# mynameisfiber/baton

Measured on NVIDIA H100. Metric: federated local samples/sec (whole box), ResNet-18 FedAvg, synthetic non-IID 32x32 shards, higher is better.
Workload: dtype bf16

## Files before the change

baton_b200/csrc/bindings.cpp:

```cpp
#include <ATen/cuda/CUDAContext.h>
#include <c10/cuda/CUDAGuard.h>
#include <torch/extension.h>

#include <optional>
#include <vector>

#include "launch.h"

namespace {

inline cudaStream_t cur_stream() { return at::cuda::getCurrentCUDAStream().stream(); }
inline void check(int rc, const char* what) {
  TORCH_CHECK(rc == 0, "baton_b200::", what, " failed with code ", rc,
              rc > 0 ? std::string(" (") + cudaGetErrorString(static_cast<cudaError_t>(rc)) + ")" : std::string());
}
inline const void* cptr(const at::Tensor& t) { return t.data_ptr(); }
inline void* ptr(at::Tensor& t) { return t.data_ptr(); }
template <class T>
inline T* opt_ptr(const std::optional<at::Tensor>& t) {
  return (t.has_value() && t->defined()) ? reinterpret_cast<T*>(t->data_ptr()) : nullptr;
}
#define CHECK_CUDA(x) TORCH_CHECK((x).is_cuda(), #x " must be a CUDA tensor")

inline const float* prox_anchor(const std::optional<at::Tensor>& anchor, int64_t numel, const at::Tensor& hyper) {
// ... 239 lines not shown
                                static_cast<int>(stride), dgrad ? 1 : 0, static_cast<int>(mc), opt_ptr<float>(col_stats),
                                cur_stream());
  if (rc == -2) return false;
  check(rc, "conv_halo");
  return true;
}
bool conv_igemm_dgrad_s2(const at::Tensor& dy, const at::Tensor& w, at::Tensor dx, int64_t kh, int64_t kw,
                         const std::vector<int64_t>& ntaps, const std::vector<int64_t>& taps, int64_t force_bn) {
  CHECK_CUDA(dy); CHECK_CUDA(w); CHECK_CUDA(dx);
  TORCH_CHECK(dy.scalar_type() == at::kBFloat16 && w.scalar_type() == at::kBFloat16 && dx.scalar_type() == at::kBFloat16 &&
              dy.dim() == 4 && dx.dim() == 4 && dy.is_contiguous() && w.is_contiguous() && dx.is_contiguous());
  TORCH_CHECK(ntaps.size() == 4 && taps.size() == 16, "conv_igemm_dgrad_s2: 4 classes x 4 taps");
  int nt[4], tw[16];
  for (int i = 0; i < 4; ++i) nt[i] = static_cast<int>(ntaps[i]);
  for (int i = 0; i < 16; ++i) tw[i] = static_cast<int>(taps[i]);
  const c10::cuda::CUDAGuard guard(dy.device());
  const int rc = b200_conv_igemm_dgrad_s2(cptr(dy), cptr(w), ptr(dx), static_cast<int>(dx.size(0)),
                                          static_cast<int>(dx.size(1)), static_cast<int>(dx.size(2)),
                                          static_cast<int>(dx.size(3)), static_cast<int>(dy.size(3)), static_cast<int>(kh),
                                          static_cast<int>(kw), static_cast<int>(dy.size(1)), static_cast<int>(dy.size(2)),
                                          nt, tw, static_cast<int>(force_bn), cur_stream());
  if (rc == -2) return false;
  check(rc, "conv_igemm_dgrad_s2");
  return true;
}
bool conv_igemm_wgrad(const at::Tensor& dy, const at::Tensor& x, at::Tensor dw, int64_t cout, int64_t kh, int64_t kw,
                      int64_t stride, int64_t pad, int64_t ho, int64_t wo, int64_t split_k, int64_t force_bn,
                      const std::optional<at::Tensor>& sgd_theta, const std::optional<at::Tensor>& sgd_theta_bf16,
                      const std::optional<at::Tensor>& sgd_mom, const std::optional<at::Tensor>& sgd_hyper,
                      bool sgd_nesterov, const std::optional<at::Tensor>& sgd_anchor,
                      const std::optional<at::Tensor>& sgd_corr, const std::optional<at::Tensor>& sgd_v) {
  CHECK_CUDA(dy); CHECK_CUDA(x); CHECK_CUDA(dw);
  TORCH_CHECK(x.scalar_type() == at::kBFloat16 && dy.scalar_type() == at::kBFloat16 && dw.scalar_type() == at::kFloat &&
              x.dim() == 4 && x.is_contiguous() && dy.is_contiguous());
  const c10::cuda::CUDAGuard guard(x.device());
  const std::optional<B200SgdEpilogue> sgd =
      sgd_epilogue(sgd_theta, sgd_theta_bf16, sgd_mom, sgd_hyper, sgd_nesterov, sgd_anchor, sgd_corr, sgd_v);
  const int rc = b200_conv_igemm_wgrad(cptr(dy), cptr(x), dw.data_ptr<float>(), static_cast<int>(x.size(0)),
                                       static_cast<int>(x.size(1)), static_cast<int>(x.size(2)), static_cast<int>(x.size(3)),
                                       static_cast<int>(cout), static_cast<int>(kh), static_cast<int>(kw),
                                       static_cast<int>(stride), static_cast<int>(pad), static_cast<int>(ho),
                                       static_cast<int>(wo), static_cast<int>(split_k), static_cast<int>(force_bn),
                                       sgd ? &*sgd : nullptr, cur_stream());
  if (rc == -2 || rc == B200_SGD_EPILOGUE_DECLINED) return false;
  check(rc, "conv_igemm_wgrad");
  return true;
// ... 886 lines not shown
  const c10::cuda::CUDAGuard guard(pred.device());
  const int in32 = pred.scalar_type() == at::kFloat;
  const int out32 = dpred.has_value() && dpred->defined() && dpred->scalar_type() == at::kFloat;
  check(b200_mse(pred.data_ptr(), in32, target.data_ptr<float>(), opt_ptr<void>(dpred), out32,
                 loss_acc.data_ptr<float>(), pred.numel(), static_cast<float>(grad_scale), cur_stream()),
        "mse");
}

}

PYBIND11_MODULE(TORCH_EXTENSION_NAME, m) {
  m.doc() = "baton_b200 sm_90a kernels";
  m.attr("MAX_RANKS") = B200_MAX_RANKS;
  m.def("gemm", &gemm);
  m.def("trace_set", &trace_set);
  m.def("attention_fwd", &attention_fwd);
  m.def("attention_bwd", &attention_bwd);
  m.def("bn_bwd_cluster", &bn_bwd_cluster);
  m.def("im2col_tma_probe", &im2col_tma_probe);
  m.def("conv_igemm_fwd", &conv_igemm_fwd);
  m.def("conv_igemm_wgrad", &conv_igemm_wgrad);
  m.def("conv_igemm_dgrad", &conv_igemm_dgrad);
  m.def("conv_igemm_dgrad_s2", &conv_igemm_dgrad_s2);
  m.def("conv_halo", &conv_halo);
  m.def("gemm_batched", &gemm_batched);
  m.def("gemm_fp8", &gemm_fp8);
  m.def("quant_mx_rows", &quant_mx_rows);
  m.def("quant_mx_cols", &quant_mx_cols);
  m.def("fused_sgd", &fused_sgd);
  m.def("fused_sgd_segments", &fused_sgd_segments);
  m.def("weighted_sum", &weighted_sum);
  m.def("fold_client", &fold_client);
  m.def("scaffold_corr", &scaffold_corr);
  m.def("scaffold_dc", &scaffold_dc);
  m.def("cast", &cast);
  m.def("gather_rows", &gather_rows);
  m.def("gather_augment", &gather_augment);
  m.def("gather_mix", &gather_mix);
  m.def("colsum", &colsum);
  m.def("add_bf16", &add_bf16);
  m.def("relu_bwd", &relu_bwd);
  m.def("gelu", &gelu);
  m.def("gelu_bwd", &gelu_bwd);
  m.def("pad_rows", &pad_rows);
  m.def("embedding_bwd", &embedding_bwd);
  m.def("fedavg_allreduce", &fedavg_allreduce);
// ... 41 lines not shown
```

baton_b200/csrc/gemm_wgmma.cu:

```cuda
#define B200_TU_TAG 1
#include "ptx.cuh"
#include "epilogue.cuh"
#include "launch.h"
#include "pdl.cuh"
#include "sgd.cuh"

namespace b200 {

constexpr int BM = 128;
constexpr int BK = 64;
constexpr int WG_K = 16;
constexpr int GEMM_THREADS = 384;
constexpr int CONSUMER_WARPS = 8;
constexpr int CONSUMER_THREADS = 32 * CONSUMER_WARPS;
constexpr int MAX_STAGES = 8;
constexpr int S2_MAX_TAPS = 4;

struct GemmParams {
  int M, N, K;
  void* D;
  long long ldd;
  const float* bias;
  int out_fp32;
  int act;
// ... 339 lines not shown
  return w;
}
__device__ __forceinline__ int s2_dx_row(const GemmParams& p, int cls, int m) {
  if (m >= p.M) return -1;
  const int hw = p.conv_ho * p.conv_wo;
  const int n = m / hw, r = m - n * hw;
  const int i = r / p.conv_wo, j = r - i * p.conv_wo;
  const int h = 2 * i + (cls >> 1), w = 2 * j + (cls & 1);
  return (h < p.conv_h && w < p.conv_w) ? (n * p.conv_h + h) * p.conv_w + w : -1;
}
template <int BN>
__device__ __forceinline__ void s2_load_ktile(const CUtensorMap* tmA, const CUtensorMap* tmB, const GemmParams& p,
                                              uint8_t* sa, uint8_t* sb, uint64_t* bar, int cls, int kt, int m0, int n0) {
  const int cblocks = p.conv_cin >> 6;
  const int slot = kt / cblocks, cb = kt - slot * cblocks;
  const int tw = s2_tap(p, cls, slot);
  const int q0 = m0 % p.conv_wo, t0 = m0 / p.conv_wo;
  tma_load_im2col_4d(sa, tmA, bar, cb * 64, q0, t0 % p.conv_ho, t0 / p.conv_ho, (tw >> 24) & 0xff, (tw >> 16) & 0xff);
  const int wcol = (tw & 0xffff) * p.conv_ncol + n0;
#pragma unroll
  for (int j = 0; j < BN / 64; ++j) tma_load_2d(sb + j * 8192, tmB, bar, wcol + j * 64, cb * 64);
}

template <int BN, int STAGES, int CONV = 0, bool SGD = false, bool AFFINE = false, bool PROX = false, bool SCAF = false,
          bool ADAM = false>
__global__ void __launch_bounds__(GEMM_THREADS, 1)
gemm_bf16_fixed_kernel(const __grid_constant__ CUtensorMap tmA, const __grid_constant__ CUtensorMap tmB,
                         const GemmParams p) {
  using L = SmemLayout<BN>;
  static_assert(STAGES * L::STAGE_BYTES >= L::PART_BYTES, "the drained ring must hold the fp32 accumulator tile");
  extern __shared__ __align__(1024) uint8_t smem_raw[];
  uint8_t* smem = reinterpret_cast<uint8_t*>((reinterpret_cast<uintptr_t>(smem_raw) + 1023) & ~uintptr_t(1023));
  uint64_t* full_bar = reinterpret_cast<uint64_t*>(smem + STAGES * L::STAGE_BYTES);
  uint64_t* empty_bar = full_bar + STAGES;
  float* cstat = reinterpret_cast<float*>(empty_bar + STAGES);

  griddep_launch_dependents();
  const int warp = threadIdx.x >> 5;
  int m0 = blockIdx.y * BM;
  const int cls = CONV == 4 ? s2_class(p, m0) : 0;
  const int n0 = blockIdx.x * BN;
  const int k_tiles_total = CONV == 4 ? s2_ntaps(p, cls) * (p.conv_cin >> 6) : (p.K + BK - 1) / BK;
  const int bz_outer = p.batched ? static_cast<int>(blockIdx.z) / p.batch_inner : 0;
  const int bz_inner = p.batched ? static_cast<int>(blockIdx.z) % p.batch_inner : 0;
  const int kt_begin = p.batched ? 0 : blockIdx.z * p.k_tiles_per_split;
  int kt_end = kt_begin + p.k_tiles_per_split;
  if (kt_end > k_tiles_total) kt_end = k_tiles_total;
  const int num_kt = kt_end - kt_begin;

  if (warp == 0 && elect_one()) {
    tma_prefetch_desc(&tmA);
    tma_prefetch_desc(&tmB);
    for (int s = 0; s < STAGES; ++s) {
      mbar_init(&full_bar[s], 1);
      mbar_init(&empty_bar[s], CONSUMER_WARPS);
    }
    fence_barrier_init();
  }
  __syncthreads();
  griddep_wait();

  if (warp == 0) {
    if (elect_one()) {
      if (p.tile_flags != nullptr) {
        const int rows_here = (p.N - n0) < BN ? (p.N - n0) : BN;
// ... 17 lines not shown
        if constexpr (CONV == 2) {
          const int live = (p.N - n0 + 63) / 64 < BN / 64 ? (p.N - n0 + 63) / 64 : BN / 64;
          mbar_expect_tx(&full_bar[s], L::A_BYTES + live * 8192);
        } else {
          mbar_expect_tx(&full_bar[s], L::STAGE_BYTES);
        }
        if (p.batched) {
          if (!p.a_mn) {
            tma_load_4d(sa, &tmA, &full_bar[s], k0, m0, bz_inner, bz_outer);
          } else {
#pragma unroll
            for (int j = 0; j < BM / 64; ++j)
              tma_load_4d(sa + j * 8192, &tmA, &full_bar[s], m0 + j * 64, k0, bz_inner, bz_outer);
          }
          if (!p.b_mn) {
            tma_load_4d(sb, &tmB, &full_bar[s], k0, n0, bz_inner, bz_outer);
          } else {
#pragma unroll
            for (int j = 0; j < BN / 64; ++j)
              tma_load_4d(sb + j * 8192, &tmB, &full_bar[s], n0 + j * 64, k0, bz_inner, bz_outer);
          }
        } else if constexpr (CONV == 4) {
          s2_load_ktile<BN>(&tmA, &tmB, p, sa, sb, &full_bar[s], cls, kt_begin + i, m0, n0);
        } else {
        if constexpr (CONV == 1 || CONV == 3) {
          const int kt = kt_begin + i;
          const int cblocks = p.conv_cin >> 6;
          const int tap = kt / cblocks, cb = kt - tap * cblocks;
          const int fr = tap / p.conv_kw, fs = tap - fr * p.conv_kw;
          const int q0 = m0 % p.conv_wo, t0 = m0 / p.conv_wo;
          tma_load_im2col_4d(sa, &tmA, &full_bar[s], cb * 64, q0 * p.conv_stride - p.conv_pad,
                             (t0 % p.conv_ho) * p.conv_stride - p.conv_pad, t0 / p.conv_ho, fs, fr);
        } else if (!p.a_mn) {
          tma_load_2d(sa, &tmA, &full_bar[s], k0, m0);
        } else {
#pragma unroll
          for (int j = 0; j < BM / 64; ++j)
            tma_load_2d(sa + j * 8192, &tmA, &full_bar[s], m0 + j * 64, k0);
        }
        if constexpr (CONV == 2) {
          const int q0 = k0 % p.conv_wo, t0 = k0 / p.conv_wo;
          const int w0 = q0 * p.conv_stride - p.conv_pad, h0 = (t0 % p.conv_ho) * p.conv_stride - p.conv_pad;
          const int img = t0 / p.conv_ho;
#pragma unroll
          for (int j = 0; j < BN / 64; ++j) {
            const int col = n0 + j * 64;
// ... 15 lines not shown
        } else {
#pragma unroll
          for (int j = 0; j < BN / 64; ++j) tma_load_2d(sb + j * 8192, &tmB, &full_bar[s], n0 + j * 64, k0);
        }
        }
      }
    }
  } else if (warp >= 4) {
    const int ew = warp - 4;
    float acc[BN / 2];
    int s = 0;
    uint32_t ph = 0;
    consume_ktiles<BN>(acc, smem, STAGES, full_bar, empty_bar, s, ph, num_kt, p.a_mn, p.b_mn, ew >> 2);
    if (threadIdx.x == 128) TRACE_POINT();
    named_bar_sync(1, CONSUMER_THREADS);
    float* part = reinterpret_cast<float*>(smem);
    wg_store_acc<BN>(acc, part, L::PART_PITCH, 64 * (ew >> 2));
    named_bar_sync(1, CONSUMER_THREADS);
    const int q = ew & 3;
    constexpr int NCHUNK = BN / 32;
    const int c_begin = (ew < 4 ? 0 : (NCHUNK + 1) / 2) * 32, c_end = (ew < 4 ? (NCHUNK + 1) / 2 : NCHUNK) * 32;
    const int lrow = q * 32 + static_cast<int>(lane_id());
    const int row = m0 + lrow;
    const int orow = CONV == 4 ? s2_dx_row(p, cls, row) : row;
    const bool row_ok = CONV == 4 ? orow >= 0 : row < p.M;
    const size_t elt = p.out_fp32 ? 4 : 2;
    uint8_t* drow = reinterpret_cast<uint8_t*>(p.D) +
                    (static_cast<size_t>(CONV == 4 && orow < 0 ? 0 : orow) * p.ldd + static_cast<size_t>(bz_outer) * p.d_outer +
                     static_cast<size_t>(bz_inner) * p.d_inner) * elt;
    const bool vec_ok = ((reinterpret_cast<uintptr_t>(p.D) & 15) == 0) && ((p.ldd * elt) % 16 == 0);
    const bool sgd_vec = SGD && (p.ldd % 4 == 0) &&
                         ((reinterpret_cast<uintptr_t>(p.sgd_theta) | reinterpret_cast<uintptr_t>(p.sgd_mom) |
                           (PROX ? reinterpret_cast<uintptr_t>(p.sgd_anchor) : 0) |
                           (SCAF ? reinterpret_cast<uintptr_t>(p.sgd_corr) : 0) |
                           (ADAM ? reinterpret_cast<uintptr_t>(p.sgd_v) : 0)) & 15) == 0 &&
                         (reinterpret_cast<uintptr_t>(p.sgd_wb) & 7) == 0;
    float* sstat = cstat + q * 2 * BN;
    const bool want_stats = p.col_stats != nullptr;
#pragma unroll 1
    for (int c = c_begin; c < c_end; c += 32) {
      uint32_t r[32];
      acc_ld_row32(part + lrow * L::PART_PITCH + c, r);
      const int col0 = n0 + c;
      float v[32];
#pragma unroll
      for (int j = 0; j < 32; ++j) v[j] = __uint_as_float(r[j]);
      if (col0 >= p.N) {
        if (want_stats) { sstat[c + lane_id()] = 0.f; sstat[BN + c + lane_id()] = 0.f; }
        continue;
      }
      if constexpr (AFFINE) {
// ... 230 lines not shown
      epilogue_tile<BN>(p, acc_tile, ew & 3, ew >> 2, m0, n0, epi_stage + ew * EPI_WARP_BYTES,
                        vec_ok && ((d_off * elt) & 15) == 0, d_off);
    }
  }
}


template <int BN, bool CLUSTER, int CONV = 0, bool AFFINE = false>
__global__ void __launch_bounds__(GEMM_THREADS, 1)
gemm_bf16_splitk_kernel(const __grid_constant__ CUtensorMap tmA, const __grid_constant__ CUtensorMap tmB,
                        const GemmParams p) {
  using L = SmemLayout<BN>;
  extern __shared__ __align__(1024) uint8_t smem_raw[];
  uint8_t* smem = reinterpret_cast<uint8_t*>((reinterpret_cast<uintptr_t>(smem_raw) + 1023) & ~uintptr_t(1023));
  const int STAGES = p.stages;
  const int ring_bytes = STAGES * L::STAGE_BYTES;
  const int data_bytes = L::PART_BYTES > ring_bytes ? L::PART_BYTES : ring_bytes;
  uint64_t* full_bar = reinterpret_cast<uint64_t*>(smem + data_bytes);
  uint64_t* empty_bar = full_bar + MAX_STAGES;
  float* cstat = reinterpret_cast<float*>(empty_bar + MAX_STAGES);

  griddep_launch_dependents();
  const int warp = threadIdx.x >> 5;
  const int m0 = blockIdx.y * BM;
  const int n0 = blockIdx.x * BN;
  const int k_tiles_total = (p.K + BK - 1) / BK;
  const int kt_begin = blockIdx.z * p.k_tiles_per_split;
  int kt_end = kt_begin + p.k_tiles_per_split;
  if (kt_end > k_tiles_total) kt_end = k_tiles_total;
  const int num_kt = kt_end - kt_begin;

  if (warp == 0 && elect_one()) {
    tma_prefetch_desc(&tmA);
    tma_prefetch_desc(&tmB);
    for (int s = 0; s < STAGES; ++s) {
      mbar_init(&full_bar[s], 1);
      mbar_init(&empty_bar[s], CONSUMER_WARPS);
    }
    fence_barrier_init();
  }
  __syncthreads();
  griddep_wait();

  if (warp == 0) {
    if (elect_one()) {
      if (p.tile_flags != nullptr) {
        const int rows_here = (p.N - n0) < BN ? (p.N - n0) : BN;
        const uint32_t need = p.flag_epoch_ptr != nullptr ? *reinterpret_cast<const volatile uint32_t*>(p.flag_epoch_ptr)
                                                          : p.flag_epoch;
        wait_arrival_flags(p.tile_flags, p.flag_elem_off + static_cast<long long>(n0) * p.ldb,
                           p.flag_elem_off + static_cast<long long>(n0 + rows_here) * p.ldb - 1, p.flag_tile_elems, need);
        if (p.flag_bias_off >= 0)
          wait_arrival_flags(p.tile_flags, p.flag_bias_off + n0, p.flag_bias_off + n0 + rows_here - 1,
                             p.flag_tile_elems, need);
        fence_proxy_async_all();
      }
      int s = 0;
      uint32_t ph = 0;
      for (int i = 0; i < num_kt; ++i) {
        mbar_wait(&empty_bar[s], ph ^ 1);
        uint8_t* sa = smem + s * L::STAGE_BYTES;
        uint8_t* sb = sa + L::A_BYTES;
        const int k0 = (kt_begin + i) * BK;
        mbar_expect_tx(&full_bar[s], L::STAGE_BYTES);
        if constexpr (CONV == 1 || CONV == 3) {
          const int kt = kt_begin + i;
          const int cblocks = p.conv_cin >> 6;
          const int tap = kt / cblocks, cb = kt - tap * cblocks;
          const int fr = tap / p.conv_kw, fs = tap - fr * p.conv_kw;
          const int q0 = m0 % p.conv_wo, t0 = m0 / p.conv_wo;
          tma_load_im2col_4d(sa, &tmA, &full_bar[s], cb * 64, q0 * p.conv_stride - p.conv_pad,
                             (t0 % p.conv_ho) * p.conv_stride - p.conv_pad, t0 / p.conv_ho, fs, fr);
        } else if (!p.a_mn) {
          tma_load_2d(sa, &tmA, &full_bar[s], k0, m0);
        } else {
#pragma unroll
          for (int j = 0; j < BM / 64; ++j)
            tma_load_2d(sa + j * 8192, &tmA, &full_bar[s], m0 + j * 64, k0);
        }
        if constexpr (CONV == 3) {
          const int kt = kt_begin + i;
          const int cblocks = p.conv_cin >> 6;
          const int tap = kt / cblocks, cb = kt - tap * cblocks;
          const int wcol = (p.conv_taps - 1 - tap) * p.conv_ncol + n0;
#pragma unroll
          for (int j = 0; j < BN / 64; ++j) tma_load_2d(sb + j * 8192, &tmB, &full_bar[s], wcol + j * 64, cb * 64);
        } else if (!p.b_mn) {
// ... 12 lines not shown
    uint32_t ph = 0;
    consume_ktiles<BN>(acc, smem, STAGES, full_bar, empty_bar, s, ph, num_kt, p.a_mn, p.b_mn, ew >> 2);
    named_bar_sync(1, CONSUMER_THREADS);
    float* part = reinterpret_cast<float*>(smem);
    wg_store_acc<BN>(acc, part, L::PART_PITCH, 64 * (ew >> 2));
    if constexpr (!CLUSTER) {
      named_bar_sync(1, CONSUMER_THREADS);
      const int q = ew & 3;
      constexpr int NCHUNK = BN / 32;
      const int c_begin = (ew < 4 ? 0 : (NCHUNK + 1) / 2) * 32, c_end = (ew < 4 ? (NCHUNK + 1) / 2 : NCHUNK) * 32;
      const int lrow = q * 32 + static_cast<int>(lane_id());
      const int row = m0 + lrow;
      const size_t elt = p.out_fp32 ? 4 : 2;
      const bool vec_ok = ((reinterpret_cast<uintptr_t>(p.D) & 15) == 0) && ((p.ldd * elt) % 16 == 0);
#pragma unroll 1
      for (int c = c_begin; c < c_end; c += 32) {
        const int col0 = n0 + c;
        if (row >= p.M || col0 >= p.N) continue;
        uint32_t r[32];
        acc_ld_row32(part + lrow * L::PART_PITCH + c, r);
        float v[32];
#pragma unroll
        for (int j = 0; j < 32; ++j) v[j] = __uint_as_float(r[j]);
        store_row_chunk<32, AFFINE>(p, row, col0, v, vec_ok);
      }
    }
  }

  if constexpr (CLUSTER) {
    const int S = p.cluster_k;
    cluster_sync_all();
    if (warp >= 4 && warp < 8) {
      const uint32_t me = cluster_ctarank();
      const int rows_per = BM / S;
      constexpr int CG = BN / 8;
      const int t = threadIdx.x - 128;
      const size_t elt = p.out_fp32 ? 4 : 2;
      const bool vec_ok = ((reinterpret_cast<uintptr_t>(p.D) & 15) == 0) && ((p.ldd * elt) % 16 == 0);
      const bool want_stats = p.col_stats != nullptr;
      float cs[8] = {0.f, 0.f, 0.f, 0.f, 0.f, 0.f, 0.f, 0.f}, cq[8] = {0.f, 0.f, 0.f, 0.f, 0.f, 0.f, 0.f, 0.f};
      for (int item = t; item < rows_per * CG; item += 128) {
        const int lrow = static_cast<int>(me) * rows_per + item / CG;
        const int c = (item % CG) * 8;
        const uint32_t laddr = smem_u32(smem) + static_cast<uint32_t>((lrow * L::PART_PITCH + c) * 4);
        float v[8] = {0.f, 0.f, 0.f, 0.f, 0.f, 0.f, 0.f, 0.f};
        for (int r = 0; r < S; ++r) {
          const float4 a = ld_dsmem_f4(laddr, r), b = ld_dsmem_f4(laddr + 16, r);
          v[0] += a.x; v[1] += a.y; v[2] += a.z; v[3] += a.w;
          v[4] += b.x; v[5] += b.y; v[6] += b.z; v[7] += b.w;
        }
        const int row = m0 + lrow, col0 = n0 + c;
        if (want_stats) {
#pragma unroll
          for (int j = 0; j < 8; ++j) {
            const float rnd = __bfloat162float(__float2bfloat16_rn(v[j]));
            cs[j] += rnd;
            cq[j] = fmaf(rnd, rnd, cq[j]);
          }
        }
        if (row < p.M && col0 < p.N) store_row_chunk<8, AFFINE>(p, row, col0, v, vec_ok);
      }
      if (want_stats) {
#pragma unroll
        for (int j = 0; j < 8; ++j) {
#pragma unroll
          for (int o = CG; o < 32; o <<= 1) {
            cs[j] += __shfl_xor_sync(0xffffffffu, cs[j], o);
            cq[j] += __shfl_xor_sync(0xffffffffu, cq[j], o);
          }
        }
        const int wq = t >> 5, ln = t & 31;
        if (ln < CG) {
#pragma unroll
          for (int j = 0; j < 8; ++j) {
            cstat[wq * 2 * BN + ln * 8 + j] = cs[j];
            cstat[wq * 2 * BN + BN + ln * 8 + j] = cq[j];
          }
        }
        named_bar_sync(2, 128);
        for (int i = t; i < 2 * BN; i += 128) {
          const int col = i < BN ? i : i - BN;
          if (n0 + col < p.N) {
            const float v = cstat[i] + cstat[2 * BN + i] + cstat[4 * BN + i] + cstat[6 * BN + i];
// ... 467 lines not shown
  }
  if (max_taps == 0) return -2;
  const int bn = clamp_bn(force_bn > 0 ? force_bn : (Cin > 64 ? 128 : 64));
  CUtensorMap ta, tb;
  int rc = b200_encode_map_im2col_bf16(&ta, dy, N, Ho, Wo, Cout, 1, 1, 1, 0, 64, BM);
  if (rc) return rc;
  rc = make_map(&tb, w, Cout, static_cast<long long>(KH) * KW * Cin, static_cast<long long>(KH) * KW * Cin, 64, BK);
  if (rc) return rc;
  const int k_tiles = max_taps * (Cout / 64);
  p.M = static_cast<int>(M); p.N = Cin; p.K = k_tiles * BK; p.D = dx; p.ldd = Cin; p.bias = nullptr; p.out_fp32 = 0;
  p.act = 0; p.a_mn = 0; p.b_mn = 1; p.k_tiles_per_split = k_tiles; p.cluster_k = 1; p.atomic_out = 0;
  p.col_stats = nullptr;
  p.tile_flags = nullptr; p.flag_epoch = 0; p.alpha = 1.0f; p.flag_elem_off = 0; p.flag_tile_elems = 0;
  p.ldb = static_cast<long long>(KH) * KW * Cin;
  p.flag_bias_off = -1; p.flag_epoch_ptr = nullptr;
  p.batched = 0; p.batch_inner = 1; p.batch_count = 1; p.d_outer = 0; p.d_inner = 0;
  p.conv_ho = Ho; p.conv_wo = Wo; p.conv_stride = 2; p.conv_pad = 0; p.conv_kw = KW; p.conv_cin = Cout;
  p.conv_taps = KH * KW; p.conv_ncol = Cin; p.conv_h = H; p.conv_w = W;
  dim3 grid((Cin + bn - 1) / bn, static_cast<unsigned>(4 * tiles_m), 1);
  if (bn == 128) return launch_fixed<128, 6, 4>(ta, tb, p, grid, stream);
  return launch_fixed<64, 8, 4>(ta, tb, p, grid, stream);
}

extern "C" int b200_conv_igemm_wgrad(const void* dy, const void* x, float* dw, int N, int H, int W, int Cin, int Cout,
                                     int KH, int KW, int stride, int pad, int Ho, int Wo, int split_k, int force_bn,
                                     const B200SgdEpilogue* sgd, cudaStream_t stream) {
  using namespace b200;
  const long long Mp = static_cast<long long>(N) * Ho * Wo;
  const int Kc = KH * KW * Cin;
  if (Mp <= 0 || Cout <= 0) return 0;
  if (Cin % 64 != 0 || Cout % 8 != 0 || Mp > (1ll << 30) || (reinterpret_cast<uintptr_t>(x) & 15) ||
      (reinterpret_cast<uintptr_t>(dy) & 15) || (reinterpret_cast<uintptr_t>(dw) & 15))
    return -2;
  const int bn = clamp_bn(force_bn > 0 ? force_bn : (Kc > 64 ? 128 : 64));
  CUtensorMap ta, tb;
  int rc = make_map(&ta, dy, Mp, Cout, Cout, 64, BK);
  if (rc) return rc;
  rc = b200_encode_map_im2col_bf16(&tb, x, N, H, W, Cin, KH, KW, stride, pad, 64, 64);
  if (rc) return rc;
  const int k_tiles = static_cast<int>((Mp + BK - 1) / BK);
  if (split_k < 1) split_k = 1;
  if (split_k > k_tiles) split_k = k_tiles;
  const int per = (k_tiles + split_k - 1) / split_k;
  split_k = (k_tiles + per - 1) / per;
  if (sgd != nullptr && split_k != 1) return B200_SGD_EPILOGUE_DECLINED;
  GemmParams p;
// ... 21 lines not shown
```

baton_b200/csrc/launch.h:

```cpp
#pragma once
#include <cuda_runtime.h>
#include <stdint.h>

#define B200_MAX_RANKS 16

extern "C" {

struct B200SgdEpilogue {
  float* theta;
  void* theta_bf16;
  float* mom;
  const float* hyper;
  int nesterov;
  const float* anchor;
  const float* corr;
  float* v;
};
#define B200_SGD_EPILOGUE_DECLINED (-6)

struct B200AffineEpilogue {
  const float* scale;
  const float* shift;
  const void* residual;
  long long ldr;
// ... 1 lines not shown
};
#define B200_AFFINE_EPILOGUE_DECLINED (-7)

int b200_gemm_bf16(const void* a, const void* b, void* d, const float* bias, int M, int N, int K, long long lda,
                   long long ldb, long long ldd, int a_mn, int b_mn, int out_fp32, int act, int split_k, int accumulate,
                   float alpha, const uint32_t* tile_flags, uint32_t flag_epoch, long long flag_elem_off, int flag_tile_elems,
                   long long flag_bias_off, int force_bn, float* col_stats, const uint32_t* flag_epoch_ptr,
                   const B200SgdEpilogue* sgd, const B200AffineEpilogue* affine, cudaStream_t stream);
int b200_gemm_bf16_batched(const void* a, const void* b, void* d, int M, int N, int K, long long lda, long long ldb,
                           long long ldd, int a_mn, int b_mn, int out_fp32, int act, float alpha, int n_outer,
                           int n_inner, long long a_outer, long long a_inner, long long b_outer, long long b_inner,
                           long long d_outer, long long d_inner, int accumulate, cudaStream_t stream);
int b200_attention_fwd(const void* qkv, void* out, void* probs, int B, int S, int H, int dh, float scale,
                       cudaStream_t stream);
int b200_attention_bwd(const void* qkv, const void* dout, const void* probs, void* dqkv, int B, int S, int H, int dh,
                       float scale, cudaStream_t stream);
int b200_conv_igemm_fwd(const void* x, const void* w, void* y, int N, int H, int W, int Cin, int Cout, int KH, int KW,
                        int stride, int pad, int Ho, int Wo, int cluster_k, int force_bn, float* col_stats,
                        const B200AffineEpilogue* affine, cudaStream_t stream);
int b200_conv_igemm_dgrad(const void* dy, const void* w, void* dx, int N, int H, int W, int Cin, int Cout, int KH, int KW,
                          int pad, int Ho, int Wo, int cluster_k, int force_bn, cudaStream_t stream);
int b200_conv_igemm_dgrad_s2(const void* dy, const void* w, void* dx, int N, int H, int W, int Cin, int Cout, int KH,
                             int KW, int Ho, int Wo, const int* ntaps, const int* taps, int force_bn, cudaStream_t stream);
int b200_conv_igemm_wgrad(const void* dy, const void* x, float* dw, int N, int H, int W, int Cin, int Cout, int KH, int KW,
                          int stride, int pad, int Ho, int Wo, int split_k, int force_bn, const B200SgdEpilogue* sgd,
                          cudaStream_t stream);
int b200_conv_halo(const void* src, const void* w, void* out, int N, int H, int W, int C, int Nout, int stride,
                   int dgrad, int mc, float* col_stats, cudaStream_t stream);
int b200_im2col_tma_probe(const void* x, void* col, int N, int H, int W, int C, int KH, int KW, int stride, int pad,
                          int Ho, int Wo, cudaStream_t stream);
int b200_gemm_fp8(const void* a, const void* b, void* d, const float* bias, const void* sfa, const void* sfb, int M, int N,
                  int K, long long lda, long long ldb, long long ldd, int out_fp32, int act, int split_k, int accumulate,
                  float alpha, cudaStream_t stream);
int b200_quant_mx_rows(const void* x, void* q, void* sf, long long R, int C, long long ld_in, int Cp, cudaStream_t stream);
int b200_quant_mx_cols(const void* x, void* q, void* sf, long long R, int C, long long ld_in, long long Rp,
                       cudaStream_t stream);
int b200_gemm_simt(const void* a, const void* b, void* d, const float* bias, int M, int N, int K, long long lda,
                   long long ldb, long long ldd, int a_mn, int b_mn, int out_fp32, int act, int accumulate,
                   float alpha, cudaStream_t stream);

int b200_fused_sgd(float* w, float* g, float* mom, void* w_bf16, long long n, const float* hyper, int zero_grad,
                   int nesterov, const unsigned long long* wire_slot, const float* pack_global,
                   const float* pack_scale, long long n_pack, int wire_fp32, const float* prox_anchor,
                   const float* corr, float* adam_v, cudaStream_t stream);
int b200_fused_sgd_segments(float* w, float* g, float* mom, void* w_bf16, const long long* segments, int n_seg,
                            const float* hyper, int nesterov, const float* prox_anchor, const float* corr,
// ... 192 lines not shown
```

baton_b200/ops/functional.py:

```python
from __future__ import annotations

import collections
import functools
from typing import List, Optional, Sequence, Tuple

import torch

from ._ext import load

BF16 = torch.bfloat16
NUM_SMS = 132


def _pitch(t: torch.Tensor) -> int:
    assert t.dim() == 2 and (t.stride(1) == 1 or t.shape[1] == 1), "GEMM operand must have unit inner stride"
    return t.stride(0) if t.shape[0] > 1 else max(t.stride(0), t.shape[1])


def _tma_ok(t: torch.Tensor) -> bool:
    return t.dtype == BF16 and _pitch(t) % 8 == 0 and t.data_ptr() % 16 == 0


def pick_bn(M: int, N: int) -> int:
    m_tiles = (M + 127) // 128
# ... 387 lines not shown


def halo_smem_bytes(h: int, w: int, c: int = 64, stride: int = 1) -> int:
    ho, wo = conv_out_size(h, 3, stride, 1), conv_out_size(w, 3, stride, 1)
    box = (HALO_BM // (ho * wo)) * (stride * (ho - 1) + 3) * (stride * (wo - 1) + 3) * 128
    k_tiles = 9 * (c // 64)
    return c // 64 * round_up(box, 1024) + k_tiles * 8192 + round_up(1 + k_tiles, 16) * 8 + 4 * 64 * 4 + 1024


def halo_eligible(kh: int, kw: int, stride: int, pad: int, c: int, h: int, w: int,
                  affine: Optional[dict] = None, dgrad: bool = False) -> bool:
    if kh != 3 or kw != 3 or pad != 1 or (stride, c) not in _HALO_FORMS or (dgrad and stride != 1):
        return False
    hw = conv_out_size(h, 3, stride, 1) * conv_out_size(w, 3, stride, 1)
    return (hw <= HALO_BM and HALO_BM % hw == 0 and affine is None and
            halo_smem_bytes(h, w, c, stride) <= _HALO_MAX_SMEM)


def halo_cluster(m_rows: int) -> int:
    tiles = (m_rows + HALO_BM - 1) // HALO_BM
    return 4 if tiles % 4 == 0 else 2 if tiles % 2 == 0 else 1


def _conv_path(path: Optional[str], eligible: bool) -> str:
    if path is None:
        return "halo" if eligible else "im2col"
    if path not in ("halo", "im2col"):
        raise ValueError("path must be None, 'halo' or 'im2col', not {!r}".format(path))
    if path == "halo" and not eligible:
        raise ValueError("the halo kernel does not take this convolution (see halo_eligible)")
    return path


def conv_igemm_fwd(x: torch.Tensor, w2d: torch.Tensor, kh: int, kw: int, stride: int, pad: int,
                   col_stats: Optional[torch.Tensor] = None, affine: Optional[dict] = None,
                   cluster_k: Optional[int] = None, force_bn: int = 0,
                   out: Optional[torch.Tensor] = None, path: Optional[str] = None,
                   mc: Optional[int] = None) -> Optional[torch.Tensor]:
    n, h, w, c = x.shape
    cout = w2d.shape[0]
    if c % 64 or w2d.shape[1] != kh * kw * c or not x.is_contiguous() or not w2d.is_contiguous():
        return None
    ho, wo = conv_out_size(h, kh, stride, pad), conv_out_size(w, kw, stride, pad)
    M, K = n * ho * wo, kh * kw * c
    halo = halo_eligible(kh, kw, stride, pad, c, h, w, affine) and cout % 8 == 0
    if _conv_path(path, halo) == "halo":
        y = out if out is not None else torch.empty((M, cout), dtype=BF16, device=x.device)
        if not load().conv_halo(x, w2d, y, stride, False, mc or halo_cluster(M), col_stats):
            raise RuntimeError("conv_halo declined a convolution halo_eligible admits")
        return y
    bn = force_bn or pick_bn(M, cout)
    if cluster_k is None:
        cluster_k = pick_cluster_k(M, cout, K, bn)
    y = out if out is not None else torch.empty((M, cout), dtype=BF16, device=x.device)
    af = affine or {}
    ok = load().conv_igemm_fwd(x, w2d, y, kh, kw, stride, pad, ho, wo, cluster_k, bn, col_stats, af.get("scale"),
                               af.get("shift"), af.get("residual"), bool(af.get("relu", False)))
    return y if ok else None


S2_MAX_TAPS = 4


def conv_s2_dgrad_taps(kh: int, kw: int, pad: int, ho: int, wo: int) -> Optional[List[List[Tuple[int, int, int]]]]:
    classes = []
    for a in (0, 1):
        for b in (0, 1):
            taps = []
            for r in range(kh):
                if (a + pad - r) % 2:
                    continue
                dp = (a + pad - r) // 2
                for s in range(kw):
                    if (b + pad - s) % 2:
                        continue
                    dq = (b + pad - s) // 2
                    if dp < 0 or dq < 0:
                        return None
                    if dp < ho and dq < wo:
                        taps.append((r * kw + s, dp, dq))
            if len(taps) > S2_MAX_TAPS:
                return None
            classes.append(taps)
    return classes


def conv_igemm_dgrad(dy: torch.Tensor, w2d: torch.Tensor, in_shape, kh: int, kw: int, pad: int, stride: int = 1,
                     out: Optional[torch.Tensor] = None, path: Optional[str] = None,
                     mc: Optional[int] = None, cluster_k: Optional[int] = None) -> Optional[torch.Tensor]:
    n, h, w, c = in_shape
    cout = dy.shape[-1]
    if c % 64 or cout % 64 or w2d.shape[1] != kh * kw * c or not dy.is_contiguous() or not w2d.is_contiguous():
        return None
    if _conv_path(path, halo_eligible(kh, kw, stride, pad, cout, h, w, dgrad=True)) == "halo":
        dx = out if out is not None else torch.empty((n, h, w, c), dtype=BF16, device=dy.device)
        if not load().conv_halo(dy, w2d, dx, 1, True, mc or halo_cluster(n * h * w), None):
            raise RuntimeError("conv_halo declined a convolution halo_eligible admits")
        return dx
    if stride == 1:
        M, K = n * h * w, kh * kw * cout
        bn = pick_bn(M, c)
        dx = out if out is not None else torch.empty((n, h, w, c), dtype=BF16, device=dy.device)
        if cluster_k is None:
            cluster_k = pick_cluster_k(M, c, K, bn)
        ok = load().conv_igemm_dgrad(dy, w2d, dx, kh, kw, pad, cluster_k, bn)
        return dx if ok else None
    if stride != 2:
        return None
    ho, wo = dy.shape[1], dy.shape[2]
    classes = conv_s2_dgrad_taps(kh, kw, pad, ho, wo)
    if classes is None:
        return None
    bn = pick_bn(4 * n * ho * wo, c)
    words = [[t | dp << 16 | dq << 24 for t, dp, dq in taps] + [0] * (S2_MAX_TAPS - len(taps)) for taps in classes]
    dx = out if out is not None else torch.empty((n, h, w, c), dtype=BF16, device=dy.device)
    ok = load().conv_igemm_dgrad_s2(dy, w2d, dx, kh, kw, [len(t) for t in classes], [x for ws in words for x in ws], bn)
    return dx if ok else None


def conv_igemm_wgrad_(dy2d: torch.Tensor, x: torch.Tensor, dw2d: torch.Tensor, kh: int, kw: int, stride: int,
# ... 184 lines not shown
```

Measured before the change: 225,600.

## Add in-image-taps conv kernel that skips padded taps for tiny spatial maps

Adds a CONV==5 mode to the WGMMA GEMM kernels that, for convolutions with at most four output pixels, loads only the kernel taps that land inside the image. Each output pixel becomes its own class with a per-class tap table, so padding taps are never multiplied. Forward (non-affine) and stride-1 dgrad now route to this path by default when eligible, replacing the generic im2col path. The cost is a new code path with fixed cluster and BN choices, and more grid rows, one per output pixel.

```diff
diff --git a/baton_b200/csrc/bindings.cpp b/baton_b200/csrc/bindings.cpp
--- a/baton_b200/csrc/bindings.cpp
+++ b/baton_b200/csrc/bindings.cpp
@@ -285,6 +285,33 @@
                                           nt, tw, static_cast<int>(force_bn), cur_stream());
   if (rc == -2) return false;
   check(rc, "conv_igemm_dgrad_s2");
+  return true;
+}
+bool conv_igemm_taps(const at::Tensor& src, const at::Tensor& w, at::Tensor out, int64_t taps, bool dgrad,
+                     const std::vector<int64_t>& ntaps, const std::vector<int64_t>& tab, int64_t cluster_k,
+                     int64_t force_bn, const std::optional<at::Tensor>& col_stats) {
+  CHECK_CUDA(src); CHECK_CUDA(w); CHECK_CUDA(out);
+  TORCH_CHECK(src.scalar_type() == at::kBFloat16 && w.scalar_type() == at::kBFloat16 && out.scalar_type() == at::kBFloat16 &&
+              src.dim() == 4 && out.dim() == 4 && src.size(0) == out.size(0) && src.is_contiguous() &&
+              w.is_contiguous() && out.is_contiguous());
+  TORCH_CHECK(ntaps.size() == 4 && tab.size() == 16, "conv_igemm_taps: 4 pixels x 4 entries");
+  const int64_t c = src.size(3), nout = out.size(3);
+  TORCH_CHECK(w.numel() == taps * c * nout, "conv_igemm_taps: w must be [Cout, taps*Cin]");
+  TORCH_CHECK(!col_stats.has_value() ||
+                  (!dgrad && col_stats->scalar_type() == at::kFloat && col_stats->numel() >= 2 * nout),
+              "conv_igemm_taps: col_stats is a [2 Cout] fp32 buffer of the forward");
+  int nt[4], tw[16];
+  for (int i = 0; i < 4; ++i) nt[i] = static_cast<int>(ntaps[i]);
+  for (int i = 0; i < 16; ++i) tw[i] = static_cast<int>(tab[i]);
+  const c10::cuda::CUDAGuard guard(src.device());
+  const int rc = b200_conv_igemm_taps(cptr(src), cptr(w), ptr(out), static_cast<int>(src.size(0)),
+                                      static_cast<int>(src.size(1) * src.size(2)), static_cast<int>(c),
+                                      static_cast<int>(nout), static_cast<int>(taps),
+                                      static_cast<int>(out.size(1) * out.size(2)), dgrad ? 1 : 0, nt, tw,
+                                      static_cast<int>(cluster_k), static_cast<int>(force_bn),
+                                      opt_ptr<float>(col_stats), cur_stream());
+  if (rc == -2) return false;
+  check(rc, "conv_igemm_taps");
   return true;
 }
 bool conv_igemm_wgrad(const at::Tensor& dy, const at::Tensor& x, at::Tensor dw, int64_t cout, int64_t kh, int64_t kw,
@@ -1217,6 +1244,7 @@
   m.def("conv_igemm_wgrad", &conv_igemm_wgrad);
   m.def("conv_igemm_dgrad", &conv_igemm_dgrad);
   m.def("conv_igemm_dgrad_s2", &conv_igemm_dgrad_s2);
+  m.def("conv_igemm_taps", &conv_igemm_taps);
   m.def("conv_halo", &conv_halo);
   m.def("gemm_batched", &gemm_batched);
   m.def("gemm_fp8", &gemm_fp8);
diff --git a/baton_b200/csrc/gemm_wgmma.cu b/baton_b200/csrc/gemm_wgmma.cu
--- a/baton_b200/csrc/gemm_wgmma.cu
+++ b/baton_b200/csrc/gemm_wgmma.cu
@@ -385,6 +385,26 @@
   for (int j = 0; j < BN / 64; ++j) tma_load_2d(sb + j * 8192, tmB, bar, wcol + j * 64, cb * 64);
 }
 
+__device__ __forceinline__ int taps_out_row(const GemmParams& p, int cls, int m) {
+  return m < p.M ? m * (p.conv_ho * p.conv_wo) + cls : -1;
+}
+template <int BN>
+__device__ __forceinline__ void taps_load_ktile(const CUtensorMap* tmA, const CUtensorMap* tmB, const GemmParams& p,
+                                                uint8_t* sa, uint8_t* sb, uint64_t* bar, int cls, int kt, int m0,
+                                                int n0) {
+  const int cblocks = p.conv_cin >> 6;
+  const int slot = kt / cblocks, cb = kt - slot * cblocks;
+  const int tw = s2_tap(p, cls, slot);
+  const int tap = tw & 0xffff, src = tw >> 16;
+  tma_load_2d(sa, tmA, bar, src * p.conv_cin + cb * 64, m0);
+  if (!p.b_mn) {
+    tma_load_2d(sb, tmB, bar, tap * p.conv_cin + cb * 64, n0);
+  } else {
+#pragma unroll
+    for (int j = 0; j < BN / 64; ++j) tma_load_2d(sb + j * 8192, tmB, bar, tap * p.conv_ncol + n0 + j * 64, cb * 64);
+  }
+}
+
 template <int BN, int STAGES, int CONV = 0, bool SGD = false, bool AFFINE = false, bool PROX = false, bool SCAF = false,
           bool ADAM = false>
 __global__ void __launch_bounds__(GEMM_THREADS, 1)
@@ -401,9 +421,9 @@
   griddep_launch_dependents();
   const int warp = threadIdx.x >> 5;
   int m0 = blockIdx.y * BM;
-  const int cls = CONV == 4 ? s2_class(p, m0) : 0;
+  const int cls = CONV >= 4 ? s2_class(p, m0) : 0;
   const int n0 = blockIdx.x * BN;
-  const int k_tiles_total = CONV == 4 ? s2_ntaps(p, cls) * (p.conv_cin >> 6) : (p.K + BK - 1) / BK;
+  const int k_tiles_total = CONV >= 4 ? s2_ntaps(p, cls) * (p.conv_cin >> 6) : (p.K + BK - 1) / BK;
   const int bz_outer = p.batched ? static_cast<int>(blockIdx.z) / p.batch_inner : 0;
   const int bz_inner = p.batched ? static_cast<int>(blockIdx.z) % p.batch_inner : 0;
   const int kt_begin = p.batched ? 0 : blockIdx.z * p.k_tiles_per_split;
@@ -467,6 +487,8 @@
           }
         } else if constexpr (CONV == 4) {
           s2_load_ktile<BN>(&tmA, &tmB, p, sa, sb, &full_bar[s], cls, kt_begin + i, m0, n0);
+        } else if constexpr (CONV == 5) {
+          taps_load_ktile<BN>(&tmA, &tmB, p, sa, sb, &full_bar[s], cls, kt_begin + i, m0, n0);
         } else {
         if constexpr (CONV == 1 || CONV == 3) {
           const int kt = kt_begin + i;
@@ -528,11 +550,11 @@
     const int c_begin = (ew < 4 ? 0 : (NCHUNK + 1) / 2) * 32, c_end = (ew < 4 ? (NCHUNK + 1) / 2 : NCHUNK) * 32;
     const int lrow = q * 32 + static_cast<int>(lane_id());
     const int row = m0 + lrow;
-    const int orow = CONV == 4 ? s2_dx_row(p, cls, row) : row;
-    const bool row_ok = CONV == 4 ? orow >= 0 : row < p.M;
+    const int orow = CONV == 4 ? s2_dx_row(p, cls, row) : CONV == 5 ? taps_out_row(p, cls, row) : row;
+    const bool row_ok = CONV >= 4 ? orow >= 0 : row < p.M;
     const size_t elt = p.out_fp32 ? 4 : 2;
     uint8_t* drow = reinterpret_cast<uint8_t*>(p.D) +
-                    (static_cast<size_t>(CONV == 4 && orow < 0 ? 0 : orow) * p.ldd + static_cast<size_t>(bz_outer) * p.d_outer +
+                    (static_cast<size_t>(CONV >= 4 && orow < 0 ? 0 : orow) * p.ldd + static_cast<size_t>(bz_outer) * p.d_outer +
                      static_cast<size_t>(bz_inner) * p.d_inner) * elt;
     const bool vec_ok = ((reinterpret_cast<uintptr_t>(p.D) & 15) == 0) && ((p.ldd * elt) % 16 == 0);
     const bool sgd_vec = SGD && (p.ldd % 4 == 0) &&
@@ -809,13 +831,14 @@
 
   griddep_launch_dependents();
   const int warp = threadIdx.x >> 5;
-  const int m0 = blockIdx.y * BM;
+  int m0 = blockIdx.y * BM;
+  const int cls = CONV == 5 ? s2_class(p, m0) : 0;
   const int n0 = blockIdx.x * BN;
-  const int k_tiles_total = (p.K + BK - 1) / BK;
+  const int k_tiles_total = CONV == 5 ? s2_ntaps(p, cls) * (p.conv_cin >> 6) : (p.K + BK - 1) / BK;
   const int kt_begin = blockIdx.z * p.k_tiles_per_split;
   int kt_end = kt_begin + p.k_tiles_per_split;
   if (kt_end > k_tiles_total) kt_end = k_tiles_total;
-  const int num_kt = kt_end - kt_begin;
+  const int num_kt = kt_end > kt_begin ? kt_end - kt_begin : 0;
 
   if (warp == 0 && elect_one()) {
     tma_prefetch_desc(&tmA);
@@ -850,6 +873,11 @@
         uint8_t* sb = sa + L::A_BYTES;
         const int k0 = (kt_begin + i) * BK;
         mbar_expect_tx(&full_bar[s], L::STAGE_BYTES);
+        if constexpr (CONV == 5) {
+          taps_load_ktile<BN>(&tmA, &tmB, p, sa, sb, &full_bar[s], cls, kt_begin + i, m0, n0);
+          if (++s == STAGES) { s = 0; ph ^= 1; }
+          continue;
+        }
         if constexpr (CONV == 1 || CONV == 3) {
           const int kt = kt_begin + i;
           const int cblocks = p.conv_cin >> 6;
@@ -908,7 +936,7 @@
         float v[32];
 #pragma unroll
         for (int j = 0; j < 32; ++j) v[j] = __uint_as_float(r[j]);
-        store_row_chunk<32, AFFINE>(p, row, col0, v, vec_ok);
+        store_row_chunk<32, AFFINE>(p, CONV == 5 ? taps_out_row(p, cls, row) : row, col0, v, vec_ok);
       }
     }
   }
@@ -944,7 +972,8 @@
             cq[j] = fmaf(rnd, rnd, cq[j]);
           }
         }
-        if (row < p.M && col0 < p.N) store_row_chunk<8, AFFINE>(p, row, col0, v, vec_ok);
+        if (row < p.M && col0 < p.N)
+          store_row_chunk<8, AFFINE>(p, CONV == 5 ? taps_out_row(p, cls, row) : row, col0, v, vec_ok);
       }
       if (want_stats) {
 #pragma unroll
@@ -1458,6 +1487,61 @@
   return launch_fixed<64, 8, 4>(ta, tb, p, grid, stream);
 }
 
+extern "C" int b200_conv_igemm_taps(const void* src, const void* w, void* out, int N, int src_hw, int C, int Nout,
+                                    int taps, int out_hw, int dgrad, const int* ntaps, const int* tab, int cluster_k,
+                                    int force_bn, float* col_stats, cudaStream_t stream) {
+  using namespace b200;
+  if (N <= 0 || Nout <= 0) return 0;
+  if (C % 64 != 0 || Nout % (dgrad ? 64 : 8) != 0 || src_hw <= 0 || out_hw <= 0 || out_hw > 4 || taps <= 0 ||
+      (dgrad && col_stats != nullptr) ||
+      (reinterpret_cast<uintptr_t>(src) & 15) || (reinterpret_cast<uintptr_t>(w) & 15) ||
+      (reinterpret_cast<uintptr_t>(out) & 15))
+    return -2;
+  const long long tiles_m = (static_cast<long long>(N) + BM - 1) / BM;
+  if (out_hw * tiles_m > 65535) return -2;
+  GemmParams p;
+  int max_taps = 0;
+  for (int c = 0; c < 4; ++c) {
+    if (ntaps[c] < 0 || ntaps[c] > S2_MAX_TAPS || (c >= out_hw && ntaps[c] != 0)) return -2;
+    for (int t = 0; t < ntaps[c]; ++t) {
+      const int tw = tab[c * S2_MAX_TAPS + t];
+      if (tw < 0 || (tw & 0xffff) >= taps || (tw >> 16) >= src_hw) return -2;
+      p.s2_tap[c][t] = tw;
+    }
+    p.s2_ntaps[c] = ntaps[c];
+    max_taps = ntaps[c] > max_taps ? ntaps[c] : max_taps;
+  }
+  if (max_taps == 0) return -2;
+  const int bn = clamp_bn(force_bn > 0 ? force_bn : (Nout > 64 ? 128 : 64));
+  const long long wcols = static_cast<long long>(taps) * (dgrad ? Nout : C);
+  CUtensorMap ta, tb;
+  int rc = make_map(&ta, src, N, static_cast<long long>(src_hw) * C, static_cast<long long>(src_hw) * C, BK, BM);
+  if (rc) return rc;
+  rc = dgrad ? make_map(&tb, w, C, wcols, wcols, 64, BK) : make_map(&tb, w, Nout, wcols, wcols, BK, bn);
+  if (rc) return rc;
+  const int k_tiles = max_taps * (C / 64);
+  if (cluster_k != 1 && cluster_k != 2 && cluster_k != 4 && cluster_k != 8) return -5;
+  while (cluster_k > 1 && (cluster_k - 1) * ((k_tiles + cluster_k - 1) / cluster_k) >= k_tiles) cluster_k >>= 1;
+  const int per = (k_tiles + cluster_k - 1) / cluster_k;
+  p.M = N; p.N = Nout; p.K = k_tiles * BK; p.D = out; p.ldd = Nout; p.bias = nullptr; p.out_fp32 = 0; p.act = 0;
+  p.a_mn = 0; p.b_mn = dgrad ? 1 : 0; p.k_tiles_per_split = per; p.cluster_k = cluster_k; p.atomic_out = 0;
+  p.col_stats = col_stats;
+  p.tile_flags = nullptr; p.flag_epoch = 0; p.alpha = 1.0f; p.flag_elem_off = 0; p.flag_tile_elems = 0;
+  p.ldb = wcols; p.flag_bias_off = -1; p.flag_epoch_ptr = nullptr;
+  p.batched = 0; p.batch_inner = 1; p.batch_count = 1; p.d_outer = 0; p.d_inner = 0;
+  p.conv_ho = 1; p.conv_wo = out_hw; p.conv_stride = 1; p.conv_pad = 0; p.conv_kw = 1; p.conv_cin = C;
+  p.conv_taps = taps; p.conv_ncol = Nout;
+  const int max_stages = bn == 128 ? 6 : 8;
+  p.stages = per < max_stages ? (per < 2 ? 2 : per) : max_stages;
+  dim3 grid((Nout + bn - 1) / bn, static_cast<unsigned>(out_hw * tiles_m), cluster_k);
+  if (cluster_k > 1) {
+    if (bn == 128) return launch_cfg<128, 5>(ta, tb, p, grid, stream);
+    return launch_cfg<64, 5>(ta, tb, p, grid, stream);
+  }
+  if (bn == 128) return launch_fixed<128, 6, 5>(ta, tb, p, grid, stream);
+  return launch_fixed<64, 8, 5>(ta, tb, p, grid, stream);
+}
+
 extern "C" int b200_conv_igemm_wgrad(const void* dy, const void* x, float* dw, int N, int H, int W, int Cin, int Cout,
                                      int KH, int KW, int stride, int pad, int Ho, int Wo, int split_k, int force_bn,
                                      const B200SgdEpilogue* sgd, cudaStream_t stream) {
diff --git a/baton_b200/csrc/launch.h b/baton_b200/csrc/launch.h
--- a/baton_b200/csrc/launch.h
+++ b/baton_b200/csrc/launch.h
@@ -47,6 +47,9 @@
                           int pad, int Ho, int Wo, int cluster_k, int force_bn, cudaStream_t stream);
 int b200_conv_igemm_dgrad_s2(const void* dy, const void* w, void* dx, int N, int H, int W, int Cin, int Cout, int KH,
                              int KW, int Ho, int Wo, const int* ntaps, const int* taps, int force_bn, cudaStream_t stream);
+int b200_conv_igemm_taps(const void* src, const void* w, void* out, int N, int src_hw, int C, int Nout, int taps,
+                         int out_hw, int dgrad, const int* ntaps, const int* tab, int cluster_k, int force_bn,
+                         float* col_stats, cudaStream_t stream);
 int b200_conv_igemm_wgrad(const void* dy, const void* x, float* dw, int N, int H, int W, int Cin, int Cout, int KH, int KW,
                           int stride, int pad, int Ho, int Wo, int split_k, int force_bn, const B200SgdEpilogue* sgd,
                           cudaStream_t stream);
diff --git a/baton_b200/ops/functional.py b/baton_b200/ops/functional.py
--- a/baton_b200/ops/functional.py
+++ b/baton_b200/ops/functional.py
@@ -433,14 +433,64 @@
     return 4 if tiles % 4 == 0 else 2 if tiles % 2 == 0 else 1
 
 
-def _conv_path(path: Optional[str], eligible: bool) -> str:
+def _conv_path(path: Optional[str], eligible: bool, taps: bool = False) -> str:
     if path is None:
-        return "halo" if eligible else "im2col"
-    if path not in ("halo", "im2col"):
-        raise ValueError("path must be None, 'halo' or 'im2col', not {!r}".format(path))
+        return "halo" if eligible else "taps" if taps else "im2col"
+    if path not in ("halo", "taps", "im2col"):
+        raise ValueError("path must be None, 'halo', 'taps' or 'im2col', not {!r}".format(path))
     if path == "halo" and not eligible:
         raise ValueError("the halo kernel does not take this convolution (see halo_eligible)")
+    if path == "taps" and not taps:
+        raise ValueError("the in-image-taps kernel does not take this convolution (see conv_pixel_taps)")
     return path
+
+
+S2_MAX_TAPS = 4
+TAPS_BN = 64
+TAPS_FWD_CLUSTER = 4
+TAPS_DGRAD_CLUSTER = 2
+TAPS_MAX_PIXELS = 4
+
+
+def conv_pixel_taps(kh: int, kw: int, stride: int, pad: int, h: int, w: int, c: int, cout: int,
+                    dgrad: bool = False) -> Optional[List[List[Tuple[int, int]]]]:
+    if c % 64 or cout % 64 or (dgrad and stride != 1) or h * w == 1:
+        return None
+    ho, wo = conv_out_size(h, kh, stride, pad), conv_out_size(w, kw, stride, pad)
+    if ho < 1 or wo < 1:
+        return None
+    oh, ow = (h, w) if dgrad else (ho, wo)
+    if oh * ow > TAPS_MAX_PIXELS:
+        return None
+    pixels = []
+    for a in range(oh):
+        for b in range(ow):
+            entries = []
+            if dgrad:
+                for i in range(ho):
+                    for j in range(wo):
+                        r, s = a - i + pad, b - j + pad
+                        if 0 <= r < kh and 0 <= s < kw:
+                            entries.append((r * kw + s, i * wo + j))
+                entries.sort(key=lambda e: kh * kw - 1 - e[0])
+            else:
+                for r in range(kh):
+                    for s in range(kw):
+                        y, x = stride * a + r - pad, stride * b + s - pad
+                        if 0 <= y < h and 0 <= x < w:
+                            entries.append((r * kw + s, y * w + x))
+            if len(entries) > S2_MAX_TAPS:
+                return None
+            pixels.append(entries)
+    if all(len(e) == kh * kw for e in pixels):
+        return None
+    return pixels
+
+
+def _taps_words(pixels: List[List[Tuple[int, int]]]) -> Tuple[List[int], List[int]]:
+    pixels = pixels + [[]] * (TAPS_MAX_PIXELS - len(pixels))
+    words = [[t | src << 16 for t, src in e] + [0] * (S2_MAX_TAPS - len(e)) for e in pixels]
+    return [len(e) for e in pixels], [x for ws in words for x in ws]
 
 
 def conv_igemm_fwd(x: torch.Tensor, w2d: torch.Tensor, kh: int, kw: int, stride: int, pad: int,
@@ -455,10 +505,19 @@
     ho, wo = conv_out_size(h, kh, stride, pad), conv_out_size(w, kw, stride, pad)
     M, K = n * ho * wo, kh * kw * c
     halo = halo_eligible(kh, kw, stride, pad, c, h, w, affine) and cout % 8 == 0
-    if _conv_path(path, halo) == "halo":
+    pixels = conv_pixel_taps(kh, kw, stride, pad, h, w, c, cout) if affine is None else None
+    kind = _conv_path(path, halo, pixels is not None)
+    if kind == "halo":
         y = out if out is not None else torch.empty((M, cout), dtype=BF16, device=x.device)
         if not load().conv_halo(x, w2d, y, stride, False, mc or halo_cluster(M), col_stats):
             raise RuntimeError("conv_halo declined a convolution halo_eligible admits")
+        return y
+    if kind == "taps":
+        y = out if out is not None else torch.empty((M, cout), dtype=BF16, device=x.device)
+        if not load().conv_igemm_taps(x, w2d, y.view(n, ho, wo, cout), kh * kw, False, *_taps_words(pixels),
+                                      TAPS_FWD_CLUSTER if cluster_k is None else cluster_k, force_bn or TAPS_BN,
+                                      col_stats):
+            raise RuntimeError("conv_igemm_taps declined a convolution conv_pixel_taps admits")
         return y
     bn = force_bn or pick_bn(M, cout)
     if cluster_k is None:
@@ -468,9 +527,6 @@
     ok = load().conv_igemm_fwd(x, w2d, y, kh, kw, stride, pad, ho, wo, cluster_k, bn, col_stats, af.get("scale"),
                                af.get("shift"), af.get("residual"), bool(af.get("relu", False)))
     return y if ok else None
-
-
-S2_MAX_TAPS = 4
 
 
 def conv_s2_dgrad_taps(kh: int, kw: int, pad: int, ho: int, wo: int) -> Optional[List[List[Tuple[int, int, int]]]]:
@@ -503,10 +559,18 @@
     cout = dy.shape[-1]
     if c % 64 or cout % 64 or w2d.shape[1] != kh * kw * c or not dy.is_contiguous() or not w2d.is_contiguous():
         return None
-    if _conv_path(path, halo_eligible(kh, kw, stride, pad, cout, h, w, dgrad=True)) == "halo":
+    pixels = conv_pixel_taps(kh, kw, stride, pad, h, w, c, cout, dgrad=True)
+    kind = _conv_path(path, halo_eligible(kh, kw, stride, pad, cout, h, w, dgrad=True), pixels is not None)
+    if kind == "halo":
         dx = out if out is not None else torch.empty((n, h, w, c), dtype=BF16, device=dy.device)
         if not load().conv_halo(dy, w2d, dx, 1, True, mc or halo_cluster(n * h * w), None):
             raise RuntimeError("conv_halo declined a convolution halo_eligible admits")
+        return dx
+    if kind == "taps":
+        dx = out if out is not None else torch.empty((n, h, w, c), dtype=BF16, device=dy.device)
+        if not load().conv_igemm_taps(dy, w2d, dx, kh * kw, True, *_taps_words(pixels),
+                                      TAPS_DGRAD_CLUSTER if cluster_k is None else cluster_k, TAPS_BN, None):
+            raise RuntimeError("conv_igemm_taps declined a convolution conv_pixel_taps admits")
         return dx
     if stride == 1:
         M, K = n * h * w, kh * kw * cout
```

Result: faster. 231,200, median of 6 (+2.5%).
